# ConsenSys/wittgenstein

Hardware: NVIDIA H100
Metric: simulated-ms/sec, GSFSignature 65,536 nodes (higher is better)
Workload: dtype u64 bitmaps / int32

## Files before the change

### wittgenstein_b200/csrc/wtg_cuda.cu

```cuda
#include <cuda_runtime.h>
#include <unistd.h>

#include <cstdio>
#include <cstdlib>
#include <stdexcept>
#include <string>
#include <vector>

#include "wtg_engine.hpp"

namespace wtg {

#define CUDA_OK(x)                                                                                       \
  do {                                                                                                   \
    cudaError_t e_ = (x);                                                                                \
    if (e_ != cudaSuccess) throw std::runtime_error(std::string("CUDA: ") + cudaGetErrorString(e_) + " at " #x); \
  } while (0)

constexpr int SCAN_THREADS = 256;
constexpr int SCAN_ITEMS = 4;
constexpr int SCAN_TILE = SCAN_THREADS * SCAN_ITEMS;

__global__ void k_begin(Dev d, int mode) {
  if (threadIdx.x >= 32) return;
  if (d.ffwd && mode == 1) {
    CoopWarp c;
    tickBeginFfwd(d, c);
  } else if (d.farCap > 0 && !d.ffwd) {
    CoopWarp c;
    tickBeginFar(d, c, mode);
  } else if (threadIdx.x == 0) {
    tickBegin(d, mode);
  }
}
__global__ void k_end(Dev d, int mode) {
  if (threadIdx.x == 0) tickEnd(d, mode);
}

__device__ __forceinline__ void listAppend(const Dev& d, bool active, int n, int* cnt, int* list, u64* words = nullptr, u64 word = 0) {
  CoopWarp c;
  unsigned m = c.ballot(active);
  if (!m) return;
  int stripe = ((blockIdx.x * blockDim.x + threadIdx.x) >> 5) & (ARENA_STRIPES - 1);
  int base = 0;
  if (c.lane() == 0) base = atomicAdd(&cnt[stripe], c.count(m));
  base = c.bcast(base, 0);
  if (active) {
    size_t at = (size_t)stripe * d.listStripeCap + base + c.rank(m);
    list[at] = n;
    if (words) words[at] = word;
  }
}
__global__ void __launch_bounds__(256) k_cond_mark(Dev d) {
  if (d.ctl->error) return;
  const int blk = blockIdx.x;
  int n = d.n0 + blk * blockDim.x + threadIdx.x;
  bool due = false;
  if (n < d.n0 + d.nLoc) due = d.proto == PROTO_HANDEL ? hCondMark(d, n) : gsfCondMark(d, n);
  listAppend(d, due, n, d.ctl->dueCnt, d.dueList);
}
template <int PHASE>
__global__ void __launch_bounds__(256) k_cond_nodes(Dev d) {
  extern __shared__ uint32_t keepAll[];
  __shared__ HScratch scratch[8];
  if (d.ctl->error) return;
  const int blk = blockIdx.x, nBlk = gridDim.x;
  const int stripe = blk & (ARENA_STRIPES - 1);
  const int cnt = d.ctl->dueCnt[stripe];
  const int warp = threadIdx.x >> 5;
  const int sub = (blk >> 6) * 8 + warp;
  const int nsub = (nBlk >> 6) * 8;
  const int* list = d.dueList + (size_t)stripe * d.listStripeCap;
  CoopWarp c;
  for (int t = sub; t < cnt; t += nsub) {
    int n = list[t];
    if (PHASE == 0) {
      if (d.proto == PROTO_HANDEL)
        hCondScanQueue(d, c, n);
      else
        gsfCondScanQueue(d, c, n);
    } else {
      if (d.proto == PROTO_HANDEL)
        hCondSelect(d, c, n, &scratch[warp]);
      else
        gsfCondSelect(d, c, n, keepAll + (size_t)warp * (size_t)(d.qcap / 32));
    }
  }
}
__global__ void __launch_bounds__(256) k_cond_score(Dev d) {
  if (d.ctl->error) return;
  const int blk = blockIdx.x, nBlk = gridDim.x;
  const int per = d.workCap / ARENA_STRIPES;
  const int stripe = blk & (ARENA_STRIPES - 1);
  int cnt = d.ctl->workCnt[stripe];
  if (cnt > per) cnt = per;
  const int warpsPerBlock = blockDim.x >> 5;
  const int sub = (blk >> 6) * warpsPerBlock + (threadIdx.x >> 5);
  const int nsub = (nBlk >> 6) * warpsPerBlock;
  CoopWarp c;
  const uint32_t* wl = d.workList + (size_t)stripe * per;
  for (int t = sub; t < cnt; t += nsub) {
    uint32_t it = wl[t];
    if (d.proto == PROTO_HANDEL)
      hScoreItem(d, c, it);
    else
      gsfScoreItem(d, c, it);
  }
}
__global__ void k_hpick_check(Dev d) {
  if (d.ctl->error) return;
  const int blk = blockIdx.x, nBlk = gridDim.x;
  for (int n = d.n0 + blk * blockDim.x + threadIdx.x; n < d.n0 + d.nLoc; n += nBlk * blockDim.x)
    if (d.hCandK[n] > 0 && hCondPick(d, n, (u64)d.hDrawBase[n], false) > d.condDraws[n]) d.ctl->hReject = 1;
}
__global__ void k_hpick_apply(Dev d) {
  if (d.ctl->error) return;
  const int blk = blockIdx.x, nBlk = gridDim.x;
  if (!d.ctl->hReject) {
    for (int n = d.n0 + blk * blockDim.x + threadIdx.x; n < d.n0 + d.nLoc; n += nBlk * blockDim.x) hCondPick(d, n, (u64)d.hDrawBase[n], true);
  } else if (blk == 0 && threadIdx.x == 0) {
    u64 idx = 0;
    for (int n = d.n0; n < d.n0 + d.nLoc; ++n) idx += (u64)hCondPick(d, n, idx, true);
  }
}

__global__ void k_dispatch_count(Dev d) {
  if (d.ctl->error) return;
  const int blk = blockIdx.x, nBlk = gridDim.x;
  int nEv = d.ctl->nEv;
  if (d.allCap > 0) {
    CoopWarp c;
    int gw = (blk * blockDim.x + threadIdx.x) >> 5, nw = (nBlk * blockDim.x) >> 5;
    for (int i = gw; i < nEv; i += nw) dispatchCountCoop(d, c, i);
    return;
  }
  for (int i = blk * blockDim.x + threadIdx.x; i < nEv; i += nBlk * blockDim.x) dispatchCount(d, i);
}
__global__ void k_dispatch_scatter(Dev d) {
  if (d.ctl->error) return;
  const int blk = blockIdx.x, nBlk = gridDim.x;
  int nEv = d.ctl->nEv;
  if (d.allCap > 0) {
    CoopWarp c;
    int gw = (blk * blockDim.x + threadIdx.x) >> 5, nw = (nBlk * blockDim.x) >> 5;
    for (int i = gw; i < nEv; i += nw) dispatchScatterCoop(d, c, i);
    return;
  }
  for (int i = blk * blockDim.x + threadIdx.x; i < nEv; i += nBlk * blockDim.x) dispatchScatter(d, i);
}

__global__ void __launch_bounds__(256) k_node_msgs(Dev d) {
  if (d.ctl->error) return;
  const int blk = blockIdx.x;
  int n = d.n0 + blk * blockDim.x + threadIdx.x;
  int flag = 0;
  u64 word = ~0ULL;
  if (n < d.n0 + d.nLoc && d.inboxFill[n] > 0) {
    CoopSerial cs;
    if (d.proto == PROTO_SANFERMIN || d.proto == PROTO_CAPPOS)
      nodeProcess(d, cs, n, 0);
    else if (d.proto == PROTO_GSF || d.proto == PROTO_PINGPONG) {
      u64 w = 0;
      int tasks = nodeProcess(d, cs, n, 1, &w);
      flag = tasks > 0 ? 1 : 0;
      if (tasks == 1) word = w;
    }
    else if (d.proto == PROTO_CASPER) {
      const u64* in = d.inbox + d.inboxOff[n];
      const Ev* bucket = d.buckets + (size_t)(d.ctl->tick & (d.ring - 1)) * (size_t)d.bcap;
      int cnt = d.inboxFill[n];
      bool simple = true;
      for (int r = 0; r < cnt && simple; ++r) {
        const Ev& ev = bucket[inboxEntry(in[r])];
        uint32_t meta = ev.kind == EV_MULTI ? d.rec[ev.aux].meta : ev.meta;
        simple = (ev.kind == EV_MSG || ev.kind == EV_MULTI) && meta == CM_ATT;
      }
      if (simple)
        nodeProcess(d, cs, n, 0);
      else
        flag = 1;
    } else
      flag = 1;
  }
  listAppend(d, flag != 0, n, d.ctl->taskCnt, d.taskList, d.taskWord, word);
}
__global__ void __launch_bounds__(256, 3) k_node_tasks(Dev d) {
  if (d.ctl->error) return;
  const int blk = blockIdx.x, nBlk = gridDim.x;
  const bool split = d.proto == PROTO_GSF || d.proto == PROTO_PINGPONG;
  const int stripe = blk & (ARENA_STRIPES - 1);
  const int cnt = d.ctl->taskCnt[stripe];
  const int sub = (blk >> 6) * 8 + (threadIdx.x >> 5);
  const int nsub = (nBlk >> 6) * 8;
  const int* list = d.taskList + (size_t)stripe * d.listStripeCap;
  const u64* words = d.taskWord + (size_t)stripe * d.listStripeCap;
  CoopWarp c;
  for (int t = sub; t < cnt; t += nsub) {
    const int n = list[t];
    const u64 w = words[t];
    if (split && w != ~0ULL)
      nodeSingleTask(d, c, n, w);
    else
      nodeProcess(d, c, n, split ? 2 : 0);
  }
}
__global__ void k_casper_fixups(Dev d) {
  const int blk = blockIdx.x;
  if (d.ctl->error || blk != 0 || threadIdx.x >= 32) return;
  CoopWarp c;
  if (d.cRandomTies && d.ctl->tieCnt > 0) casperResolveTies(d, c);
  if (d.G == 1 && d.cg->createdThisTick > 1) casperRenumber(d, c);
}
__device__ __forceinline__ Pair pairAdd(Pair x, Pair y) {
  Pair r;
  r.a = x.a + y.a;
// ... 406 lines not shown
    const char* g = std::getenv("WTG_NO_GRAPH");
    if (g && g[0] == '1') useGraph = false;
  }
  ~CudaBackend() override {
    for (void* q : ipcOpened) cudaIpcCloseMemHandle(q);
    if (tickGraph) cudaGraphExecDestroy(tickGraph);
    if (st) cudaStreamDestroy(st);
  }
  void* alloc(size_t bytes) override {
    bind();
    void* p = nullptr;
    cudaError_t e = cudaMalloc(&p, bytes);
    if (e != cudaSuccess) throw std::runtime_error("cudaMalloc of " + std::to_string(bytes) + " bytes failed: " + cudaGetErrorString(e));
    CUDA_OK(cudaMemsetAsync(p, 0, bytes, st));
    return p;
  }
  void release(void* p) override { cudaFree(p); }
  int deviceId() const override { return devId; }
  void exportShared(void* p, unsigned char* handle) override {
    bind();
    std::memset(handle, 0, 128);
    cudaIpcMemHandle_t ih;
    CUDA_OK(cudaIpcGetMemHandle(&ih, p));
    static_assert(sizeof(ih) == 64, "cudaIpcMemHandle_t");
    std::memcpy(handle, &ih, 64);
    long long pid = (long long)getpid();
    std::memcpy(handle + 64, &pid, 8);
    std::memcpy(handle + 72, &p, sizeof(p));
    std::memcpy(handle + 80, &devId, 4);
  }
  std::vector<void*> ipcOpened;
  void* importShared(const unsigned char* handle) override {
    bind();
    long long pid;
    void* p;
    int dev;
    std::memcpy(&pid, handle + 64, 8);
    std::memcpy(&p, handle + 72, sizeof(p));
    std::memcpy(&dev, handle + 80, 4);
    if (pid == (long long)getpid()) {
      if (dev != devId) {
        int can = 0;
        CUDA_OK(cudaDeviceCanAccessPeer(&can, devId, dev));
        if (!can) throw std::runtime_error("GPU " + std::to_string(devId) + " cannot access GPU " + std::to_string(dev) + " (peer access)");
        cudaError_t e = cudaDeviceEnablePeerAccess(dev, 0);
        if (e != cudaSuccess && e != cudaErrorPeerAccessAlreadyEnabled) CUDA_OK(e);
        cudaGetLastError();
      }
      return p;
    }
    cudaIpcMemHandle_t ih;
    std::memcpy(&ih, handle, 64);
    void* q = nullptr;
    CUDA_OK(cudaIpcOpenMemHandle(&q, ih, cudaIpcMemLazyEnablePeerAccess));
    ipcOpened.push_back(q);
    return q;
  }
  void upload(void* dst, const void* src, size_t bytes) override {
    bind();
    CUDA_OK(cudaMemcpyAsync(dst, src, bytes, cudaMemcpyHostToDevice, st));
    CUDA_OK(cudaStreamSynchronize(st));
  }
  void download(void* dst, const void* src, size_t bytes) override {
    bind();
    CUDA_OK(cudaMemcpyAsync(dst, src, bytes, cudaMemcpyDeviceToHost, st));
    CUDA_OK(cudaStreamSynchronize(st));
  }
  void sync() override {
    bind();
    CUDA_OK(cudaStreamSynchronize(st));
    drainProfile();
  }
  void timerStart() override {
    bind();
    if (!tm0) {
      CUDA_OK(cudaEventCreate(&tm0));
      CUDA_OK(cudaEventCreate(&tm1));
    }
    CUDA_OK(cudaEventRecord(tm0, st));
  }
  double timerStopMs() override {
    bind();
    CUDA_OK(cudaEventRecord(tm1, st));
    CUDA_OK(cudaEventSynchronize(tm1));
    float ms = 0;
    CUDA_OK(cudaEventElapsedTime(&ms, tm0, tm1));
    return (double)ms;
  }
  void profileEnable(bool on) override {
    sync();
    profiling = on;
    if (on) {
      for (int i = 0; i < NK; ++i) {
        profMs[i] = 0;
        profCnt[i] = 0;
      }
    }
  }
  int profileRead(double* ms, long long* cnt, const char** names, int cap) override {
    sync();
    int k = 0;
    for (int i = 0; i < NK && k < cap; ++i, ++k) {
      ms[k] = profMs[i];
      cnt[k] = profCnt[i];
      names[k] = profNames[i];
    }
    return k;
  }
  void drainProfile() {
    for (size_t i = 0; i < evUsed; ++i) {
      float ms = 0;
      cudaEventElapsedTime(&ms, evPool[2 * i], evPool[2 * i + 1]);
      profMs[evKernel[i]] += ms;
      profCnt[evKernel[i]] += 1;
    }
    evUsed = 0;
  }
  void profBegin(int kid) {
    if (!profiling) return;
    if (evUsed * 2 + 2 > evPool.size()) {
      if (evUsed >= 8192) {
        CUDA_OK(cudaStreamSynchronize(st));
        drainProfile();
      } else {
        cudaEvent_t a, b;
        CUDA_OK(cudaEventCreate(&a));
        CUDA_OK(cudaEventCreate(&b));
        evPool.push_back(a);
        evPool.push_back(b);
        evKernel.push_back(0);
      }
    }
    evKernel[evUsed] = kid;
    CUDA_OK(cudaEventRecord(evPool[2 * evUsed], st));
  }
  void profEnd() {
    if (!profiling) return;
    CUDA_OK(cudaEventRecord(evPool[2 * evUsed + 1], st));
    ++evUsed;
  }

  void enqueueTick(const Dev& d, int mode) {
    const int wide = sms * 8;
    const size_t msSmem = (size_t)d.msWarps * d.ring * sizeof(int);
    if (mode != 3) {
      profBegin(P_BEGIN);
      k_begin<<<1, 32, 0, st>>>(d, mode);
      profEnd();
    }
    if ((d.proto == PROTO_GSF || d.proto == PROTO_HANDEL) && mode != 3) {
      const size_t smem8 = d.proto == PROTO_GSF ? (size_t)8 * (size_t)(d.qcap / 32) * sizeof(uint32_t) : 0;
      profBegin(P_COND_SCAN);
      k_cond_mark<<<(d.nLoc + 255) / 256, 256, 0, st>>>(d);
      k_cond_nodes<0><<<ARENA_STRIPES * 19, 256, 0, st>>>(d);
      profEnd();
      profBegin(P_COND_SCORE);
      k_cond_score<<<ARENA_STRIPES * 19, 256, 0, st>>>(d);
      profEnd();
      profBegin(P_COND_SELECT);
      k_cond_nodes<1><<<ARENA_STRIPES * 19, 256, smem8, st>>>(d);
      profEnd();
      launches += 4;
      if (d.proto == PROTO_HANDEL) {
        profBegin(P_SCAN_PARTIAL);
        k_scan_partial<<<wide, SCAN_THREADS, 0, st>>>(d, 2);
        profEnd();
        profBegin(P_SCAN_FINAL);
        k_scan_final<<<wide, SCAN_THREADS, 0, st>>>(d, 2);
        profEnd();
        profBegin(P_COND_SELECT);
        k_hpick_check<<<sms, 256, 0, st>>>(d);
        k_hpick_apply<<<sms, 256, 0, st>>>(d);
        profEnd();
        launches += 3;
      }
    }
    if (mode != 2 && mode != 3) {
      profBegin(P_DISPATCH_COUNT);
      k_dispatch_count<<<wide, 256, 0, st>>>(d);
      profEnd();
      profBegin(P_SCAN_PARTIAL);
      k_scan_partial<<<wide, SCAN_THREADS, 0, st>>>(d, 0);
      profEnd();
      profBegin(P_SCAN_FINAL);
      k_scan_final<<<wide, SCAN_THREADS, 0, st>>>(d, 0);
      profEnd();
      profBegin(P_DISPATCH_SCATTER);
      k_dispatch_scatter<<<wide, 256, 0, st>>>(d);
      profEnd();
      profBegin(P_NODE);
      k_node_msgs<<<(d.nLoc + 255) / 256, 256, 0, st>>>(d);
      k_node_tasks<<<ARENA_STRIPES * 19, 256, 0, st>>>(d);
      if (d.proto == PROTO_CASPER) {
        k_casper_fixups<<<1, 32, 0, st>>>(d);
        launches += 1;
      }
      profEnd();
      launches += 6;
    }
    profBegin(P_SCAN_PARTIAL);
    k_scan_partial<<<wide, SCAN_THREADS, 0, st>>>(d, 1);
    profEnd();
    profBegin(P_SCAN_FINAL);
    k_scan_final<<<wide, SCAN_THREADS, 0, st>>>(d, 1);
    profEnd();
    if (d.G > 1) {
      profBegin(P_EXCHANGE);
      k_x1_publish<<<sms * 2, 256, 0, st>>>(d);
      k_x_sync<<<1, 32, 0, st>>>(d, 0);
      k_x1_totals<<<1, 1, 0, st>>>(d);
      k_x1_offsets<<<sms * 2, 256, 0, st>>>(d);
      profEnd();
      launches += 4;
    }
    profBegin(P_EMIT);
    if (d.shufCap > 0) {
      k_shuffle_check<<<ARENA_STRIPES * 4, 256, 0, st>>>(d);
      k_shuffle_serial<<<1, 1, 0, st>>>(d);
      launches += 2;
    }
    k_emit<<<ARENA_STRIPES * 16, 256, 0, st>>>(d);
    if (d.allCap > 0) {
      if (d.G > 1)
        k_x_all_publish<<<8, 128, 0, st>>>(d);
      else
        k_emit_all<<<d.allWarps / 4, 128, 0, st>>>(d);
      launches += 1;
    }
    profEnd();
    if (d.G > 1) {
      profBegin(P_EXCHANGE);
      k_x_sync<<<1, 32, 0, st>>>(d, 1);
      k_x2_ingest<<<sms * 4, 256, 0, st>>>(d);
      launches += 2;
      if (d.allCap > 0) {
        k_x_all_build<<<d.allWarps / 4, 128, 0, st>>>(d);
        launches += 1;
      }
      profEnd();
    }
    profBegin(P_MS_COUNT);
    k_ms_count<<<sms * 2, d.msWarps * 32, msSmem, st>>>(d);
    profEnd();
    profBegin(P_MS_SCAN);
    k_ms_scan<<<(d.ring + 127) / 128, 128, 0, st>>>(d);
    profEnd();
    profBegin(P_MS_SCATTER);
    k_ms_scatter<<<sms * 2, d.msWarps * 32, msSmem, st>>>(d);
    profEnd();
    const bool pooled = d.proto == PROTO_GSF || d.proto == PROTO_HANDEL;
    if (pooled) {
      profBegin(P_FREE);
      k_free<<<ARENA_STRIPES * 2, 256, 0, st>>>(d);
      profEnd();
    }
    profBegin(P_END);
    k_end<<<1, 1, 0, st>>>(d, mode);
    profEnd();
    launches += pooled ? 9 : 8;
  }
  void configure(const Dev& d) {
    const size_t msSmem = (size_t)d.msWarps * d.ring * sizeof(int);
    if (msSmem > (size_t)smemOptin) throw std::runtime_error("time ring too large for the multisplit's shared-memory histogram");
  }
  void tick(const Dev& d, int mode) override {
    bind();
    configure(d);
    enqueueTick(d, mode);
    CUDA_OK(cudaGetLastError());
  }
  void ticks(const Dev& d, int count) override {
    bind();
    configure(d);
    if (!useGraph || profiling || count < 4) {
      for (int i = 0; i < count; ++i) enqueueTick(d, 1);
      CUDA_OK(cudaGetLastError());
      return;
    }
    if (!tickGraph || graphFor != (const void*)d.ctl) {
      if (tickGraph) cudaGraphExecDestroy(tickGraph);
      cudaGraph_t g;
      long long before = launches;
      CUDA_OK(cudaStreamBeginCapture(st, cudaStreamCaptureModeThreadLocal));
      enqueueTick(d, 1);
      CUDA_OK(cudaStreamEndCapture(st, &g));
      graphKernels = launches - before;
      launches = before;
      CUDA_OK(cudaGraphInstantiate(&tickGraph, g, 0));
      cudaGraphDestroy(g);
      graphFor = (const void*)d.ctl;
    }
    for (int i = 0; i < count; ++i) CUDA_OK(cudaGraphLaunch(tickGraph, st));
    launches += graphKernels * count;
  }
  void gsfInitNodes(const Dev& d) override {
    bind();
    k_gsf_init_nodes<<<(d.nLoc + 255) / 256, 256, 0, st>>>(d);
    CUDA_OK(cudaGetLastError());
  }
  void rngCandidates(const Dev& d, unsigned long long s0, unsigned long long count, int maxBound,
                     std::vector<unsigned long long>& out) override {
    bind();
    const u64 chunk = 16384;
    u64 threads = (count + chunk - 1) / chunk;
    int cap = (int)std::min<u64>((u64)1 << 26, count / 1024 + (1 << 16));
    u64* dOut = nullptr;
    int* dCnt = nullptr;
    CUDA_OK(cudaMalloc(&dOut, (size_t)cap * sizeof(u64)));
    CUDA_OK(cudaMalloc(&dCnt, sizeof(int)));
    CUDA_OK(cudaMemsetAsync(dCnt, 0, sizeof(int), st));
    u64 blocks = (threads + 127) / 128;
    k_rng_candidates<<<(unsigned)blocks, 128, 0, st>>>(d, s0, count, chunk, maxBound, dOut, dCnt, cap);
    CUDA_OK(cudaGetLastError());
// ... 35 lines not shown
```

### wittgenstein_b200/csrc/wtg_logic.cuh

```cuda
#pragma once
#include "wtg_types.h"

template <class T, class U>
static inline T wtg_host_fetch_add(T* p, U v) {
  T o = *p;
  *p = (T)(o + (T)v);
  return o;
}
template <class T>
static inline T wtg_host_fetch_max(T* p, T v) {
  T o = *p;
  if (v > o) *p = v;
  return o;
}
template <class T>
static inline T wtg_host_fetch_min(T* p, T v) {
  T o = *p;
  if (v < o) *p = v;
  return o;
}
template <class T>
static inline T wtg_host_cas(T* p, T a, T b) {
  T o = *p;
  if (o == a) *p = b;
// ... 271 lines not shown
  const int src = (int)((meta >> META_SRC_SHIFT) & 7u);
  const int nw = poolWords(l);
  const u64 pl = ev->pl;
  uint32_t slot = 0;
  int ok = 1;
  if (c.lane() == 0) ok = poolAlloc(d, l, (int)ev->to, slot) ? 1 : 0;
  slot = (uint32_t)c.bcast((int)slot, 0);
  ok = c.bcast(ok, 0);
  if (ok) {
    const u64* from = xStagePtr(d, d.rank, src, (int)(uint32_t)pl);
    u64* dst = d.pool[l] + (size_t)slot * (size_t)nw;
    for (int w = c.lane(); w < nw; w += C::LANES) dst[w] = from[w];
  }
  c.sync();
  if (c.lane() == 0) {
    ev->meta = meta & ~(META_STAGED | (7u << META_SRC_SHIFT));
    ev->pl = (pl & 0xFFFFFFFF00000000ULL) | (u64)slot;
    if (!ok) d.newTarget[g] = -1;
  }
  c.sync();
}
WTG_HD bool xNeedsIngest(const Dev& d, int g) {
  return d.proto == PROTO_GSF && d.newTarget[g] >= 0 && d.newEv[g].kind == EV_MSG && (d.newEv[g].meta & META_STAGED) != 0;
}

WTG_HD int gsfScoreFrom(int l, int size, int cV, int cSig, bool inter, int cWI, int cWIV, bool interIndiv) {
  int newTotal, added;
  if (cV == 0) {
    newTotal = cSig;
    added = cSig;
  } else if (inter) {
    newTotal = cWI;
    added = cWI - cV;
  } else {
    newTotal = cWIV;
    added = cWIV - cV;
  }
  if (added <= 0) return (cSig == 1 && !interIndiv) ? 1 : 0;
  if (newTotal == size) return 1000000 - l * 10;
  return 100000 - l * 100 + added;
}

WTG_HD int gsfScoreScalarC(const Dev& d, int n, const QEntry& e, int cV, int cI, int cU);
WTG_HD int gsfScoreScalar(const Dev& d, int n, const QEntry& e) {
  int l = (int)metaLevel(e.meta);
  return gsfScoreScalarC(d, n, e, d.cntVer[n * d.L + l], d.cntIndiv[n * d.L + l], d.cntUnion[n * d.L + l]);
}
WTG_HD int gsfScoreScalarC(const Dev& d, int n, const QEntry& e, int cV, int cI, int cU) {
  int l = (int)metaLevel(e.meta);
  int kind = (int)metaKind(e.meta);
  int size = 1 << (l - 1);
  if (cV >= size) return 0;
  const u64* rowV = d.verified + (size_t)n * d.W64;
  const u64* rowI = d.indivVer + (size_t)n * d.W64;
  if (kind == PK_FULL) {
    int k = (int)metaK(e.meta);
    int c = 1 << k;
    bool interIndiv = cI > 0;
    return gsfScoreFrom(l, size, cV, c, cV > 0, c, c, interIndiv);
  }
  if (kind == PK_INDIV) {
    int f = (int)e.from;
    bool inV = (rowV[f >> 6] >> (f & 63)) & 1ULL;
    bool inI = (rowI[f >> 6] >> (f & 63)) & 1ULL;
    return gsfScoreFrom(l, size, cV, 1, inV, cI + (inI ? 0 : 1), cU + ((inI || inV) ? 0 : 1), inI);
  }
  Blk b = levelBlock((int)e.from, l);
  u64 s = e.pl, v = rowV[b.w0] & b.mask, i = rowI[b.w0] & b.mask;
  return gsfScoreFrom(l, size, cV, WTG_POPC64(s), (s & v) != 0, WTG_POPC64(i | s), WTG_POPC64(i | s | v), (s & i) != 0);
}

template <class C>
WTG_HD void poolCounts(C& c, const u64* sig, const u64* rowV, const u64* rowI, int nw, int& cWI, int& cWIV, int& inter, int& interI) {
  for (int w = c.lane(); w < nw; w += C::LANES) {
    u64 s = sig[w], v = rowV[w], i = rowI[w];
    cWI += WTG_POPC64(i | s);
    cWIV += WTG_POPC64(i | s | v);
    inter |= (s & v) != 0;
    interI |= (s & i) != 0;
  }
}
#if defined(__CUDACC__)
__device__ __forceinline__ void poolCounts(CoopWarp& c, const u64* sig, const u64* rowV, const u64* rowI, int nw, int& cWI, int& cWIV,
                                           int& inter, int& interI) {
  const ulonglong2* s2 = reinterpret_cast<const ulonglong2*>(sig);
  const ulonglong2* v2 = reinterpret_cast<const ulonglong2*>(rowV);
  const ulonglong2* i2 = reinterpret_cast<const ulonglong2*>(rowI);
  const int n2 = nw >> 1;
  for (int w0 = c.lane(); w0 < n2; w0 += 128) {
    ulonglong2 sv[4], vv[4], iv[4];
#pragma unroll
    for (int u = 0; u < 4; ++u) {
      int w = w0 + 32 * u;
      if (w < n2) {
        sv[u] = s2[w];
        vv[u] = v2[w];
        iv[u] = i2[w];
      } else {
        sv[u] = make_ulonglong2(0, 0);
        vv[u] = sv[u];
        iv[u] = sv[u];
      }
    }
#pragma unroll
    for (int u = 0; u < 4; ++u) {
      cWI += __popcll(iv[u].x | sv[u].x) + __popcll(iv[u].y | sv[u].y);
      cWIV += __popcll(iv[u].x | sv[u].x | vv[u].x) + __popcll(iv[u].y | sv[u].y | vv[u].y);
      inter |= ((sv[u].x & vv[u].x) | (sv[u].y & vv[u].y)) != 0;
      interI |= ((sv[u].x & iv[u].x) | (sv[u].y & iv[u].y)) != 0;
    }
  }
}
#endif

template <class C>
WTG_HD int gsfScorePool(const Dev& d, C& c, int n, uint32_t from, uint32_t meta, u64 pl) {
  int l = (int)metaLevel(meta);
  int size = 1 << (l - 1);
  int cV = d.cntVer[n * d.L + l];
  if (cV >= size) return 0;
  Blk b = levelBlock((int)from, l);
  const u64* rowV = d.verified + (size_t)n * d.W64 + b.w0;
  const u64* rowI = d.indivVer + (size_t)n * d.W64 + b.w0;
  const u64* sig = d.pool[l] + (size_t)(uint32_t)pl * (size_t)b.nw;
  int cWI = 0, cWIV = 0, inter = 0, interI = 0;
  poolCounts(c, sig, rowV, rowI, b.nw, cWI, cWIV, inter, interI);
  cWI = c.sum(cWI);
  cWIV = c.sum(cWIV);
  bool bi = c.any(inter != 0), bii = c.any(interI != 0);
  return gsfScoreFrom(l, size, cV, (int)(pl >> 32), bi, cWI, cWIV, bii);
}

WTG_HD bool gsfCondMark(const Dev& d, int n) {
  const Ctl& ctl = *d.ctl;
  bool dueNow = false;
  if (ctl.condMode != 0 && !d.ndown[n]) {
    int ms = d.minStart[n];
    bool due = ctl.condMode == 1 ? (ms <= ctl.tick) : (ms <= ctl.until);
    if (due && d.stamp[n] != ctl.callId) {
      d.stamp[n] = ctl.callId;
      if (d.qLen[n] > 0) {
        dueNow = true;
        d.minStart[n] = ctl.tick + d.pairing[n];
        statAdd(d, n, ST_CONDRUNS, 1ULL);
      }
    }
  }
  d.condDue[n] = dueNow ? 1 : 0;
  if (!dueNow) d.condFired[n] = 0;
  return dueNow;
}

constexpr int COND_UNROLL = 4;
template <class C>
WTG_HD void gsfCondScanQueue(const Dev& d, C& c, int n) {
  int len = d.qLen[n];
  QEntry* q = d.queue + (size_t)n * d.qcap;
  int* qsc = d.qScore + (size_t)n * d.qcap;
  uint32_t* qst = d.qStamp + (size_t)n * d.qcap;
  const uint32_t* ver = d.lvVer + (size_t)n * d.L;
  const int st = n & (ARENA_STRIPES - 1);
  const int per = d.workCap / ARENA_STRIPES;
  int reeval = 0;
  const int myL = c.lane() < d.L ? c.lane() : 0;
  const int verMine = (int)ver[myL];
  const int cvMine = d.cntVer[n * d.L + myL], ciMine = d.cntIndiv[n * d.L + myL], cuMine = d.cntUnion[n * d.L + myL];
  for (int base0 = 0; base0 < len; base0 += C::LANES * COND_UNROLL) {
    QEntry e[COND_UNROLL];
    uint32_t es[COND_UNROLL];
#pragma unroll
    for (int u = 0; u < COND_UNROLL; ++u) {
      int i = base0 + u * C::LANES + c.lane();
      if (i < len) {
        e[u] = q[i];
        es[u] = qst[i];
      } else {
        e[u].from = 0;
        e[u].meta = 0;
        e[u].pl = 0;
        es[u] = 0;
      }
    }
#pragma unroll
    for (int u = 0; u < COND_UNROLL; ++u) {
      int i = base0 + u * C::LANES + c.lane();
      bool stalePool = false;
      const int lv = (int)metaLevel(e[u].meta);
      const uint32_t v = (uint32_t)c.gather(verMine, lv, reinterpret_cast<const int*>(ver));
      const int cV = c.gather(cvMine, lv, d.cntVer + n * d.L), cI = c.gather(ciMine, lv, d.cntIndiv + n * d.L),
                cU = c.gather(cuMine, lv, d.cntUnion + n * d.L);
      if (i < len) {
        if (es[u] != v) {
          ++reeval;
          if (metaKind(e[u].meta) == PK_POOL) {
            stalePool = true;
          } else {
            qsc[i] = gsfScoreScalarC(d, n, e[u], cV, cI, cU);
            qst[i] = v;
          }
        }
      }
      uint32_t pm = c.ballot(stalePool);
      if (pm) {
        int cnt = c.count(pm), off = c.rank(pm);
        int b0 = 0;
        if (c.lane() == 0) b0 = WTG_ATOMIC_ADD(&d.ctl->workCnt[st], cnt);
        b0 = c.bcast(b0, 0);
        if (stalePool) {
          if (b0 + off < per)
            d.workList[(size_t)st * per + b0 + off] = (uint32_t)((size_t)n * d.qcap + i);
          else
            setError(d, ERR_DESC_OVERFLOW, -n);
        }
      }
    }
  }
  reeval = c.sum(reeval);
  if (c.lane() == 0) {
    statAdd(d, n, ST_EVALENTRIES, (unsigned long long)len);
    statAdd(d, n, ST_EVALPOOL, (unsigned long long)reeval);
  }
}

template <class C>
WTG_HD void gsfScoreItem(const Dev& d, C& c, uint32_t item) {
  int n = (int)(item / (uint32_t)d.qcap);
  QEntry e = d.queue[item];
  int s = gsfScorePool(d, c, n, e.from, e.meta, e.pl);
  if (c.lane() == 0) {
    d.qScore[item] = s;
    d.qStamp[item] = d.lvVer[(size_t)n * d.L + metaLevel(e.meta)];
    statAdd(d, n, ST_EVALWORDS, (unsigned long long)(3 * poolWords((int)metaLevel(e.meta))));
  }
}

template <class C>
WTG_HD void gsfCondSelect(const Dev& d, C& c, int n, uint32_t* keepBits) {
  const Ctl& ctl = *d.ctl;
  int len = d.qLen[n];
  const int pairing = d.pairing[n];
  QEntry* q = d.queue + (size_t)n * d.qcap;
  int* qsc = d.qScore + (size_t)n * d.qcap;
  uint32_t* qst = d.qStamp + (size_t)n * d.qcap;
  int bestScore = 0, bestIdx = 0x7fffffff;
  for (int base0 = 0; base0 < len; base0 += C::LANES * COND_UNROLL) {
    int sc[COND_UNROLL];
#pragma unroll
    for (int u = 0; u < COND_UNROLL; ++u) {
      int i = base0 + u * C::LANES + c.lane();
      sc[u] = i < len ? qsc[i] : 0;
    }
#pragma unroll
    for (int u = 0; u < COND_UNROLL; ++u) {
      int base = base0 + u * C::LANES;
      if (base >= len) break;
      int i = base + c.lane();
      uint32_t km = c.ballot(sc[u] > 0);
      if (c.lane() == 0) keepBits[base / C::LANES] = km;
      if (sc[u] > bestScore) {
        bestScore = sc[u];
        bestIdx = i;
      }
    }
  }
  int mx = c.maxv(bestScore);
  int bi = c.minv(bestScore == mx ? bestIdx : 0x7fffffff);
  bool found = mx > 0;
  c.sync();
  QEntry best;
  best.from = 0;
  best.meta = 0;
  best.pl = 0;
  int w = 0;
  int base0 = 0;
  for (; base0 < len; base0 += C::LANES) {
    uint32_t kw = keepBits[base0 / C::LANES];
    int inChunk = len - base0 < C::LANES ? len - base0 : C::LANES;
    int tot = c.count(kw);
    bool hasBest = found && bi >= base0 && bi < base0 + C::LANES;
    if (tot != inChunk || hasBest) break;
    w += tot;
  }
  for (; base0 < len; base0 += C::LANES * COND_UNROLL) {
    QEntry e[COND_UNROLL];
    int es[COND_UNROLL];
    uint32_t et[COND_UNROLL];
#pragma unroll
    for (int u = 0; u < COND_UNROLL; ++u) {
      int i = base0 + u * C::LANES + c.lane();
      if (i < len) {
        e[u] = q[i];
        es[u] = qsc[i];
        et[u] = qst[i];
      } else {
        e[u].from = 0;
        e[u].meta = 0;
        e[u].pl = 0;
        es[u] = 0;
        et[u] = 0;
      }
    }
    c.sync();
#pragma unroll
    for (int u = 0; u < COND_UNROLL; ++u) {
      int base = base0 + u * C::LANES;
      if (base >= len) break;
      int i = base + c.lane();
      bool keep = false, evict = false;
      uint32_t kw = keepBits[base / C::LANES];
      if (i < len) {
        bool k0 = (kw >> c.lane()) & 1u;
        keep = k0 && !(found && i == bi);
        evict = !k0;
      }
      uint32_t km = c.ballot(keep);
      int off = c.rank(km);
      int tot = c.count(km);
      if (keep && w + off != i) {
        q[w + off] = e[u];
        qsc[w + off] = es[u];
        qst[w + off] = et[u];
      }
      if (evict && metaKind(e[u].meta) == PK_POOL) freeDirect(d, (int)metaLevel(e[u].meta), (uint32_t)e[u].pl);
      if (found && i == bi) best = e[u];
      w += tot;
    }
    c.sync();
  }
  if (found) {
    int srcLane = bi % C::LANES;
    best.from = (uint32_t)c.bcast((int)best.from, srcLane);
    best.meta = (uint32_t)c.bcast((int)best.meta, srcLane);
    best.pl = c.bcast64(best.pl, srcLane);
  }
  if (c.lane() == 0) {
    d.qLen[n] = w;
    if (found) {
      WTG_ATOMIC_ADD(&d.sigChecked[n], 1);
      d.sigQueueSize[n] = w;
      Ev ev;
      ev.kind = EV_TASK;
      ev.to = (uint32_t)n;
      ev.from = best.from;
      ev.meta = best.meta;
      ev.pl = best.pl;
      ev.aux = 0;
      ev.pad = (uint32_t)d.ctl->tick + 1u;
      d.condEv[n] = ev;
      d.condTarget[n] = ctl.tick + pairing;
    }
    d.condFired[n] = found ? 1 : 0;
  }
}

template <class C>
WTG_HD int descAlloc(const Dev& d, C& c, int n, int cnt) {
  int base = 0;
  if (c.lane() == 0) {
    int st = n & (ARENA_STRIPES - 1);
    int per = d.descCap / ARENA_STRIPES;
    int i = WTG_ATOMIC_ADD(&d.ctl->descCnt[st], cnt);
    if (i + cnt > per) {
      setError(d, ERR_DESC_OVERFLOW, i + cnt);
      base = -1;
    } else {
      base = st * per + i;
    }
  }
  return c.bcast(base, 0);
}
WTG_HD int destAlloc(const Dev& d, int n, int cnt) {
  int st = n & (ARENA_STRIPES - 1);
  int per = d.destScratchCap / ARENA_STRIPES;
  int i = WTG_ATOMIC_ADD(&d.ctl->destCnt[st], cnt);
  if (i + cnt > per) {
    setError(d, ERR_DESC_OVERFLOW, i + cnt);
    return -1;
  }
  return st * per + i;
}

WTG_HD void gsfLevelCounters(const Dev& d, int n, int l, int& cV, int& cI, int& cU) {
  cV = d.cntVer[n * d.L + l];
  cI = d.cntIndiv[n * d.L + l];
  cU = d.cntUnion[n * d.L + l];
}


template <class C>
WTG_HD int gsfLastFinishedLevel(const Dev& d, C& c, int n) {
  uint32_t comp = 0;
  for (int k = 0; k < 32 / C::LANES; ++k) {
    const int l = k * C::LANES + c.lane();
    comp |= c.ballot(l >= 1 && l < d.L && d.cntVer[n * d.L + l] == (1 << (l - 1))) << (k * C::LANES);
  }
  return WTG_CTZ32(~(comp >> 1));
}

WTG_HD void gsfOnNewSig(const Dev& d, int n, uint32_t from, uint32_t meta, u64 pl) {
  int l = (int)metaLevel(meta);
  int len = d.qLen[n];
  QEntry* q = d.queue + (size_t)n * d.qcap;
  if (len + 2 > d.qcap) {
    setError(d, ERR_QUEUE_OVERFLOW, n);
    if (metaKind(meta) == PK_POOL) freeDeferred(d, n, l, (uint32_t)pl);
    return;
  }
  QEntry e;
  e.from = from;
  e.meta = meta;
  e.pl = pl;
  uint32_t* qs = d.qStamp + (size_t)n * d.qcap;
  qs[len] = 0;
  q[len++] = e;
  u64* rowS = d.indivSeen + (size_t)n * d.W64;
  u64 bit = 1ULL << (from & 63);
  if (!(rowS[from >> 6] & bit)) {
    rowS[from >> 6] |= bit;
    QEntry ie;
    ie.from = from;
    ie.meta = metaMake(PK_INDIV, (uint32_t)l, 0);
    ie.pl = 0;
    qs[len] = 0;
    q[len++] = ie;
  }
  d.qLen[n] = len;
  d.sigQueueSize[n] = len;
  statMax(d, n, ST_MAXQUEUE, (unsigned long long)len);
}

template <class C>
WTG_HD int gsfTakePeers(const Dev& d, C& c, int n, int l, int want, uint32_t* out) {
  int rem = d.remaining[n * d.L + l];
  int p = d.pos[n * d.L + l];
  int sz = 1 << (l - 1);
  int cnt = want < rem ? want : rem;
  for (int i = 0; i < cnt; ++i) {
    out[i] = peerAt(d, n, l, p);
    if (++p >= sz) p = 0;
  }
  c.sync();
  if (c.lane() == 0) {
    d.remaining[n * d.L + l] = rem - cnt;
    d.pos[n * d.L + l] = p;
  }
  c.sync();
  return cnt;
}

template <class C>
WTG_HD void gsfUpdate(const Dev& d, C& c, int n, uint32_t from, uint32_t meta, u64 pl, int item, int& outSlots, int& outDraws) {
  const int L = d.L;
  const int tick = d.ctl->tick;
  int l = (int)metaLevel(meta);
  int kind = (int)metaKind(meta);
  int k = (int)metaK(meta);
  int size = 1 << (l - 1);
  Blk b = levelBlock((int)from, l);
  u64* rowV = d.verified + (size_t)n * d.W64;
  u64* rowI = d.indivVer + (size_t)n * d.W64;
  int cV, cI, cU;
  gsfLevelCounters(d, n, l, cV, cI, cU);
  int total = d.totalCard[n];
  int cSig = kind == PK_INDIV ? 1 : kind == PK_FULL ? (1 << k) : kind == PK_INLINE ? WTG_POPC64(pl) : (int)(pl >> 32);
  if (c.lane() == 0) {
    statAdd(d, n, ST_UPDATES, 1ULL);
    WTG_ATOMIC_ADD(&d.lvVer[n * L + l], 1u);
  }

  if (cSig == 1) {
    u64 bit = 1ULL << (from & 63);
    u64 wI = rowI[from >> 6], wV = rowV[from >> 6];
    c.sync();
    if (!(wI & bit)) {
      if (c.lane() == 0) rowI[from >> 6] = wI | bit;
      cI += 1;
      if (!(wV & bit)) cU += 1;
    }
    c.sync();
  }

  bool changed = false;
  bool superset = (kind == PK_FULL && k >= l);
  if (superset) {
    bool resetRemaining = false;
    for (int i = 1; i < L && i <= k; ++i) {
      int ci = d.cntVer[n * L + i];
      int si = 1 << (i - 1);
      if (ci != si) {
        Blk wb = levelBlock(n ^ (1 << (i - 1)), i);
        for (int w = c.lane(); w < wb.nw; w += C::LANES) rowV[wb.w0 + w] |= wb.mask;
        total += si - ci;
        if (c.lane() == 0) {
          d.cntVer[n * L + i] = si;
          d.cntUnion[n * L + i] = si;
          d.lvVer[n * L + i] += 1;
        }
        if (i == l) {
          cV = si;
          cU = si;
        }
        resetRemaining = true;
      }
      if (resetRemaining && c.lane() == 0) d.remaining[n * L + i] = si;
    }
// ... 1288 lines not shown
```

Measured before the change: 4697.

## Fuse GSF condition select into scan for single-window queues without stale pools

When a node's queue fits in one unrolled warp window and has no stale pool entries, the scan phase now keeps entries, stamps and scores in registers and does the best-pick and compaction right away. It then marks condDue as 2 so the later select kernel skips that node, which avoids re-reading the queue from global memory. The condition kernels also get more blocks per stripe and a launch bound asking for 4 blocks per SM. The fused path adds register pressure in the scan kernel and relies on the condDue flag being read consistently across kernels.

```diff
diff --git a/wittgenstein_b200/csrc/wtg_cuda.cu b/wittgenstein_b200/csrc/wtg_cuda.cu
--- a/wittgenstein_b200/csrc/wtg_cuda.cu
+++ b/wittgenstein_b200/csrc/wtg_cuda.cu
@@ -20,6 +20,7 @@
 constexpr int SCAN_THREADS = 256;
 constexpr int SCAN_ITEMS = 4;
 constexpr int SCAN_TILE = SCAN_THREADS * SCAN_ITEMS;
+constexpr int COND_STRIPE_BLOCKS = 24;
 
 __global__ void k_begin(Dev d, int mode) {
   if (threadIdx.x >= 32) return;
@@ -60,7 +61,7 @@
   listAppend(d, due, n, d.ctl->dueCnt, d.dueList);
 }
 template <int PHASE>
-__global__ void __launch_bounds__(256) k_cond_nodes(Dev d) {
+__global__ void __launch_bounds__(256, 4) k_cond_nodes(Dev d) {
   extern __shared__ uint32_t keepAll[];
   __shared__ HScratch scratch[8];
   if (d.ctl->error) return;
@@ -773,13 +774,13 @@
       const size_t smem8 = d.proto == PROTO_GSF ? (size_t)8 * (size_t)(d.qcap / 32) * sizeof(uint32_t) : 0;
       profBegin(P_COND_SCAN);
       k_cond_mark<<<(d.nLoc + 255) / 256, 256, 0, st>>>(d);
-      k_cond_nodes<0><<<ARENA_STRIPES * 19, 256, 0, st>>>(d);
+      k_cond_nodes<0><<<ARENA_STRIPES * COND_STRIPE_BLOCKS, 256, 0, st>>>(d);
       profEnd();
       profBegin(P_COND_SCORE);
-      k_cond_score<<<ARENA_STRIPES * 19, 256, 0, st>>>(d);
+      k_cond_score<<<ARENA_STRIPES * COND_STRIPE_BLOCKS, 256, 0, st>>>(d);
       profEnd();
       profBegin(P_COND_SELECT);
-      k_cond_nodes<1><<<ARENA_STRIPES * 19, 256, smem8, st>>>(d);
+      k_cond_nodes<1><<<ARENA_STRIPES * COND_STRIPE_BLOCKS, 256, smem8, st>>>(d);
       profEnd();
       launches += 4;
       if (d.proto == PROTO_HANDEL) {
diff --git a/wittgenstein_b200/csrc/wtg_logic.cuh b/wittgenstein_b200/csrc/wtg_logic.cuh
--- a/wittgenstein_b200/csrc/wtg_logic.cuh
+++ b/wittgenstein_b200/csrc/wtg_logic.cuh
@@ -447,9 +447,85 @@
 }
 
 constexpr int COND_UNROLL = 4;
+
+template <class C>
+WTG_HD void gsfCondFinish(const Dev& d, C& c, int n, bool found, int bi, QEntry best, int w) {
+  const Ctl& ctl = *d.ctl;
+  if (found) {
+    int srcLane = bi % C::LANES;
+    best.from = (uint32_t)c.bcast((int)best.from, srcLane);
+    best.meta = (uint32_t)c.bcast((int)best.meta, srcLane);
+    best.pl = c.bcast64(best.pl, srcLane);
+  }
+  if (c.lane() == 0) {
+    d.qLen[n] = w;
+    if (found) {
+      WTG_ATOMIC_ADD(&d.sigChecked[n], 1);
+      d.sigQueueSize[n] = w;
+      Ev ev;
+      ev.kind = EV_TASK;
+      ev.to = (uint32_t)n;
+      ev.from = best.from;
+      ev.meta = best.meta;
+      ev.pl = best.pl;
+      ev.aux = 0;
+      ev.pad = (uint32_t)ctl.tick + 1u;
+      d.condEv[n] = ev;
+      d.condTarget[n] = ctl.tick + d.pairing[n];
+    }
+    d.condFired[n] = found ? 1 : 0;
+  }
+}
+
+template <class C>
+WTG_HD void gsfCondSelectWindow(const Dev& d, C& c, int n, int len, const QEntry* e, const uint32_t* es, const int* sc) {
+  QEntry* q = d.queue + (size_t)n * d.qcap;
+  int* qsc = d.qScore + (size_t)n * d.qcap;
+  uint32_t* qst = d.qStamp + (size_t)n * d.qcap;
+  int bestScore = 0, bestIdx = 0x7fffffff;
+#pragma unroll
+  for (int u = 0; u < COND_UNROLL; ++u) {
+    const int i = u * C::LANES + c.lane();
+    if (i < len && sc[u] > bestScore) {
+      bestScore = sc[u];
+      bestIdx = i;
+    }
+  }
+  const int mx = c.maxv(bestScore);
+  const int bi = c.minv(bestScore == mx ? bestIdx : 0x7fffffff);
+  const bool found = mx > 0;
+  c.sync();
+  QEntry best;
+  best.from = 0;
+  best.meta = 0;
+  best.pl = 0;
+  int w = 0;
+#pragma unroll
+  for (int u = 0; u < COND_UNROLL; ++u) {
+    const int base = u * C::LANES;
+    if (base >= len) break;
+    const int i = base + c.lane();
+    const bool k0 = i < len && sc[u] > 0;
+    const bool keep = k0 && !(found && i == bi), evict = i < len && !k0;
+    const uint32_t km = c.ballot(keep);
+    const int to = w + c.rank(km);
+    if (keep && to != i) {
+      q[to] = e[u];
+      qsc[to] = sc[u];
+      qst[to] = es[u];
+    }
+    if (evict && metaKind(e[u].meta) == PK_POOL) freeDirect(d, (int)metaLevel(e[u].meta), (uint32_t)e[u].pl);
+    if (found && i == bi) best = e[u];
+    w += c.count(km);
+  }
+  gsfCondFinish(d, c, n, found, bi, best, w);
+  if (c.lane() == 0) d.condDue[n] = 2;
+}
+
 template <class C>
 WTG_HD void gsfCondScanQueue(const Dev& d, C& c, int n) {
   int len = d.qLen[n];
+  const bool oneWindow = len <= C::LANES * COND_UNROLL;
   QEntry* q = d.queue + (size_t)n * d.qcap;
   int* qsc = d.qScore + (size_t)n * d.qcap;
   uint32_t* qst = d.qStamp + (size_t)n * d.qcap;
@@ -457,23 +533,27 @@
   const int st = n & (ARENA_STRIPES - 1);
   const int per = d.workCap / ARENA_STRIPES;
   int reeval = 0;
+  bool anyPool = false;
   const int myL = c.lane() < d.L ? c.lane() : 0;
   const int verMine = (int)ver[myL];
   const int cvMine = d.cntVer[n * d.L + myL], ciMine = d.cntIndiv[n * d.L + myL], cuMine = d.cntUnion[n * d.L + myL];
+  QEntry e[COND_UNROLL];
+  uint32_t es[COND_UNROLL];
+  int sc[COND_UNROLL];
   for (int base0 = 0; base0 < len; base0 += C::LANES * COND_UNROLL) {
-    QEntry e[COND_UNROLL];
-    uint32_t es[COND_UNROLL];
 #pragma unroll
     for (int u = 0; u < COND_UNROLL; ++u) {
       int i = base0 + u * C::LANES + c.lane();
       if (i < len) {
         e[u] = q[i];
         es[u] = qst[i];
+        sc[u] = oneWindow ? qsc[i] : 0;
       } else {
         e[u].from = 0;
         e[u].meta = 0;
         e[u].pl = 0;
         es[u] = 0;
+        sc[u] = 0;
       }
     }
 #pragma unroll
@@ -490,13 +570,16 @@
           if (metaKind(e[u].meta) == PK_POOL) {
             stalePool = true;
           } else {
-            qsc[i] = gsfScoreScalarC(d, n, e[u], cV, cI, cU);
+            sc[u] = gsfScoreScalarC(d, n, e[u], cV, cI, cU);
+            es[u] = v;
+            qsc[i] = sc[u];
             qst[i] = v;
           }
         }
       }
       uint32_t pm = c.ballot(stalePool);
       if (pm) {
+        anyPool = true;
         int cnt = c.count(pm), off = c.rank(pm);
         int b0 = 0;
         if (c.lane() == 0) b0 = WTG_ATOMIC_ADD(&d.ctl->workCnt[st], cnt);
@@ -515,6 +598,7 @@
     statAdd(d, n, ST_EVALENTRIES, (unsigned long long)len);
     statAdd(d, n, ST_EVALPOOL, (unsigned long long)reeval);
   }
+  if (oneWindow && !anyPool) gsfCondSelectWindow(d, c, n, len, e, es, sc);
 }
 
 template <class C>
@@ -531,9 +615,8 @@
 
 template <class C>
 WTG_HD void gsfCondSelect(const Dev& d, C& c, int n, uint32_t* keepBits) {
-  const Ctl& ctl = *d.ctl;
+  if (d.condDue[n] != 1) return;
   int len = d.qLen[n];
-  const int pairing = d.pairing[n];
   QEntry* q = d.queue + (size_t)n * d.qcap;
   int* qsc = d.qScore + (size_t)n * d.qcap;
   uint32_t* qst = d.qStamp + (size_t)n * d.qcap;
@@ -622,30 +705,7 @@
     }
     c.sync();
   }
-  if (found) {
-    int srcLane = bi % C::LANES;
-    best.from = (uint32_t)c.bcast((int)best.from, srcLane);
-    best.meta = (uint32_t)c.bcast((int)best.meta, srcLane);
-    best.pl = c.bcast64(best.pl, srcLane);
-  }
-  if (c.lane() == 0) {
-    d.qLen[n] = w;
-    if (found) {
-      WTG_ATOMIC_ADD(&d.sigChecked[n], 1);
-      d.sigQueueSize[n] = w;
-      Ev ev;
-      ev.kind = EV_TASK;
-      ev.to = (uint32_t)n;
-      ev.from = best.from;
-      ev.meta = best.meta;
-      ev.pl = best.pl;
-      ev.aux = 0;
-      ev.pad = (uint32_t)d.ctl->tick + 1u;
-      d.condEv[n] = ev;
-      d.condTarget[n] = ctl.tick + pairing;
-    }
-    d.condFired[n] = found ? 1 : 0;
-  }
+  gsfCondFinish(d, c, n, found, bi, best, w);
 }
 
 template <class C>
```

New measurement: 4703, median of 6. About the same (+0.1%).
